# nolan-h-hamilton/ROCCO

Measured on AMD Instinct MI355X. Metric: loci/sec to converged solve, hg38 50bp K=100; BED3 intervals bit-exact, higher is better.
Workload: dtype f64

## Files before the change

rocco_amd/csrc/budget.hip:

```cpp
#include "budget.h"

#include <algorithm>
#include <atomic>
#include <chrono>
#include <cmath>
#include <cstdio>
#include <cstdlib>
#include <cstring>
#include <thread>

#include "chain.h"
#include "model_chain.h"
#include "chain_fast.h"
#include "lean.h"
#include "lean_tasks.h"
#include "search.h"

namespace rocco {

namespace {

struct DevProblem {
    const double *scores = nullptr;
    const double *costs = nullptr;
// ... 959 lines not shown
    {
        const size_t at = align_up(ls.pool_at, 256);
        if (at + bytes > ls.pool_end) {
            return nullptr;
        }
        ls.pool_at = at + bytes;
        return (char *)solver_->dev_lean_pool.ptr + at;
    }

    LeanWcapSlot wcap_slot(size_t problem) const { return lean_wcap_slot(solver_->dev_lean_wcap.ptr, probs.size(), problem); }

    void add_wcap_task(DevProblem &p, const LeanWcapSlot &slot, std::vector<LeanWcapTask> &tasks, int &blocks)
    {
        if (p.wcap_version == p.map_version) {
            return;
        }
        tasks.push_back(lean_wcap_task(p.emap, p.scores, (long long)p.n, p.qexp, p.cmax, p.sabs, slot, blocks));
        blocks += lean_tiles(p.n);
        p.wcap_version = p.map_version;
    }

    int reserve_round_scratch(long long records, bool force_fill)
    {
        DeviceBuffer &look = solver_->dev_lean_look;
        const void *old_ptr = look.ptr;
        const size_t old_bytes = look.bytes;
        int rc;
        if ((rc = look.reserve(align_up(256 + (size_t)records * 4 * sizeof(unsigned long long), 256))) != ROCCO_HIP_OK) return rc;
        if (force_fill || solver_->lean_look_dirty != 0 || look.ptr != old_ptr || look.bytes != old_bytes) {
            ROCCO_HIP_TRY(hipMemsetAsync(look.ptr, 0xFF, look.bytes, stream_));
            ROCCO_HIP_TRY(hipMemsetAsync((char *)look.ptr + 128, 0, 4, stream_));
            solver_->lean_look_dirty = 0;
        }
        return solver_->dev_lean_round.reserve(align_up((size_t)records * sizeof(LeanTileRec), 256) + 256);
    }

    LeanLaunch round_launch(const LeanTask *tasks, const double *points, LeanResult *results) const
    {
        char *look = (char *)solver_->dev_lean_look.ptr;
        LeanLaunch L;
        L.tasks = tasks;
        L.n_tasks = 0;
        L.n_units = 0;
        L.points = points;
        L.ticket = (unsigned *)look;
        L.look = (unsigned long long *)(look + 256);
        L.recs = (LeanTileRec *)solver_->dev_lean_round.ptr;
        L.bits = (unsigned *)solver_->dev_lean_pool.ptr;
        L.tile_off = (unsigned *)solver_->dev_lean_pool.ptr;
        L.results = results;
        L.error = (unsigned *)(look + 128);
        L.error_out = nullptr;
        L.self_reset = 1;
        L.pad = 0;
        L.ctl = nullptr;
        return L;
    }

    static double separator_score(double base, double gamma) { return std::floor(base - 2.0 * gamma - 2.0); }

    std::vector<std::vector<std::pair<double, long long>>> facts_;
    std::vector<std::pair<size_t, double>> open_facts_;
    bool model_chain_inflight_ = false;
    bool model_chain_running_ = false;
    int model_chain_ingested_ = 0;
    std::vector<size_t> model_chain_problems_;
    const ModelChainReport *model_chain_report_ = nullptr;
    const int *model_chain_np_ = nullptr;
    const ModelChainFact *model_chain_facts_ = nullptr;
    const ModelChainFinal *model_chain_finals_ = nullptr;
    struct Written {
        bool valid = false;
        double penalty = 0.0;
        long long count = 0;
    };
    std::vector<Written> written_;
    long long model_chain_written = 0, model_chain_windows_answered = 0;
    long long model_chains = 0, model_chain_facts = 0, model_chain_hits = 0, model_chain_misses = 0, model_chain_stopped = 0;
    long long model_tiles_answered_ = 0;
    double t_mchain_submit_ = 0.0, t_mchain_wait_ = 0.0;

    std::vector<std::pair<const char *, double>> marks_;
    bool marks_on_ = false;
    void mark(const char *label)
    {
        if (marks_on_) {
            marks_.emplace_back(label, now_us());
        }
    }

    hipEvent_t staged_event_ = nullptr;
    bool staged_pending_ = false;
    ~HipEvaluator() override
    {
        if (model_chain_running_ || !objective_pending_.empty() || objective_staged_pending_ || staged_pending_) {
            (void)hipStreamSynchronize(stream_);
        }
        if (staged_event_ != nullptr) {
            (void)hipEventDestroy(staged_event_);
        }
        if (objective_staged_event_ != nullptr) {
            (void)hipEventDestroy(objective_staged_event_);
        }
    }
    int stage_wait()
    {
        if (staged_pending_) {
// ... 2129 lines not shown
```

rocco_amd/csrc/lean.h:

```cpp
#pragma once

#include "common.h"

namespace rocco {

constexpr int kLeanChunk = 32;
constexpr int kLeanThreads = 256;
constexpr int kLeanTile = kLeanChunk * kLeanThreads;
constexpr int kLeanBatch = 8;
constexpr int kLeanMaxPoints = 64;

struct LeanTileRec {
    unsigned base;
    unsigned tail;
    unsigned cells;
    unsigned flags;
};

struct LeanTask {
    const double *s;
    long long m;
    double c_raw;
    double magic;
    double big;
    int n_tiles;
    int n_points;
    int n_groups;
    int unit_begin;
    int point_begin;
    int rec_begin;
    long long bits_begin;
    long long off_begin;
    int result_begin;
    int tile_stride;
    int independent;
    int store;
    const uint8_t *emap;
    const double *wcap;
    const unsigned *clean_chunks;
    double cmax, sabs;
    int qexp;
    int batch;
};

struct LeanResult {
    long long count;
    long long child_len;
    long long flags;
};

struct LeanRoundCtl {
    int n_tasks;
    int n_units;
    int n_pairs;
    int n_pre_tasks;
    int n_pre_blocks;
    unsigned error;
    int round;
    int all_done;
};

struct LeanLaunch {
    const LeanTask *tasks;
    int n_tasks;
    int n_units;
    const double *points;
    unsigned *ticket;
    unsigned long long *look;
    LeanTileRec *recs;
    unsigned *bits;
    unsigned *tile_off;
    LeanResult *results;
    unsigned *error;
    unsigned *error_out;
    int self_reset;
    int pad;
    LeanRoundCtl *ctl;
};

struct LeanCompactTask {
    const double *s;
    const int *orig;
    long long m;
    int n_tiles;
    int block_begin;
    const unsigned *bits;
    const unsigned *tile_off;
    double sep;
    double *out_s;
    int *out_orig;
    long long capacity;
};

struct LeanWriteTask {
    const unsigned *word1;
    const unsigned *word0;
    const unsigned *entering;
    uint8_t *solution;
    long long m;
    int n_tiles;
    int block_begin;
};
int launch_lean_write_solutions(const LeanWriteTask *tasks_dev, const int *n_tasks_dev, int grid, hipStream_t stream);

struct LeanMapOut {
    double *gain_chunk;
    double *gain_block;
};
struct LeanMapCodeTask {
    const double *gain_chunk;
    const double *gain_block;
    uint8_t *emap;
    long long m;
    double margin;
    int n_tiles;
    int block_begin;
};
int launch_lean_map(const LeanLaunch &L, const LeanMapOut &out, hipStream_t stream);
int launch_lean_mapcode(const LeanMapCodeTask *tasks_dev, int n_tasks, int n_blocks, hipStream_t stream);

int launch_lean_eval(const LeanLaunch &L, hipStream_t stream);
int launch_lean_eval_chain(const LeanLaunch &L, int grid, hipStream_t stream);
int launch_lean_finish_chain(const LeanLaunch &L, int grid, hipStream_t stream);
int launch_lean_compact_chain(const LeanCompactTask *tasks_dev, LeanRoundCtl *ctl, int grid, hipStream_t stream);
constexpr int kLeanModelBatch = 4;
int launch_lean_model(const LeanLaunch &L, hipStream_t stream);
struct LeanWcapTask {
    const uint8_t *emap;
    const double *s;
// ... 27 lines not shown
```

rocco_amd/csrc/lean.hip:

```cpp
#include "lean.h"
#include "model_chain.h"

#include <cmath>

namespace rocco {

namespace {

constexpr int kStride = kLeanChunk + 2;
constexpr int kTileLds = kLeanThreads * kStride;
constexpr unsigned long long kSentinel = ~0ull;
constexpr unsigned kSpinLimit = 1u << 22;

struct Fn {
    double a, lo, hi;
};

__device__ __forceinline__ double clampd(double x, double lo, double hi) { return fmin(fmax(x, lo), hi); }

__device__ __forceinline__ Fn compose(const Fn &f, const Fn &g)
{
    Fn r;
    r.a = f.a + g.a;
    r.lo = clampd(f.lo + g.a, g.lo, g.hi);
    r.hi = clampd(f.hi + g.a, g.lo, g.hi);
    return r;
}

__device__ __forceinline__ Fn shfl_up_fn(const Fn &f, int off)
{
    Fn r;
    r.a = __shfl_up(f.a, off);
    r.lo = __shfl_up(f.lo, off);
    r.hi = __shfl_up(f.hi, off);
    return r;
}

__device__ __forceinline__ unsigned long long granule_load(const unsigned long long *p)
{
    return __hip_atomic_load(p, __ATOMIC_RELAXED, __HIP_MEMORY_SCOPE_AGENT);
}

__device__ __forceinline__ void granule_store(unsigned long long *p, double v)
{
    __hip_atomic_store(p, (unsigned long long)__double_as_longlong(v), __ATOMIC_RELAXED, __HIP_MEMORY_SCOPE_AGENT);
}

__device__ __forceinline__ double granule_wait(const unsigned long long *p, unsigned *error)
{
    unsigned long long v = granule_load(p);
    unsigned spins = 0;
    while (v == kSentinel) {
        __builtin_amdgcn_s_sleep(2);
        v = granule_load(p);
        if (++spins > kSpinLimit) {
            atomicOr(error, 1u);
            return 0.0;
        }
    }
    return __longlong_as_double((long long)v);
}

template <typename First>
__device__ __forceinline__ int find_task(int n_tasks, int key, First first_of)
{
    const int lane = threadIdx.x & 63;
    int ti = 0;
    for (int base = 0; base < n_tasks; base += 64) {
        const int i = base + lane;
        const int v = (i < n_tasks) ? first_of(i) : 0x7FFFFFFF;
        const unsigned long long le = __ballot(v <= key);
        if (le == 0ull) {
            break;
        }
        ti = base + 63 - __builtin_clzll(le);
        if (le != ~0ull) {
            break;
        }
    }
    return ti;
}

template <bool RAW>
__device__ __forceinline__ void stage_tile(const double *__restrict__ s, long long m, long long base, double magic,
                                           double *lds)
{
    const int t = threadIdx.x;
    const bool aligned16 = ((reinterpret_cast<uintptr_t>(s) & 15U) == 0);
    if (aligned16 && base + kLeanTile <= m) {
        const double2 *__restrict__ src = reinterpret_cast<const double2 *>(s + base) + t;
        double2 v[16];
#pragma unroll
        for (int r = 0; r < 16; ++r) {
            v[r] = src[r * kLeanThreads];
        }
#pragma unroll
        for (int r = 0; r < 16; ++r) {
            const int e = 2 * (r * kLeanThreads + t);
// ... 178 lines not shown
        const bool coded = code_hz || (e - 52 < task.qexp);
        const bool hz = coded || (fabs(-x[p] - lm.nlam[p]) == lm.half_u) || gamma_tie;
        lm.hz[p] = hz;
        lm.tie[p] = hz && !coded;
        lm.c[p] = hz ? cq : cu;
        lm.w[p] = hz ? (4.0 * hb + q) : 0.0;
        lm.base[p] = hz ? (9.0 * hb + 2.0 * q) : 0.0;
    }
}

template <int PB>
__device__ __forceinline__ void chunk_function_model(const double *__restrict__ row, const double (&x)[PB],
                                                     const LaneModel<PB> &lm, bool first_unclamped, double big, Fn (&f)[PB])
{
    double lo[PB], hi[PB], fa[PB];
#pragma unroll
    for (int p = 0; p < PB; ++p) {
        fa[p] = 0.0;
        lo[p] = -big;
        hi[p] = big;
    }
#pragma unroll 1
    for (int i0 = 0; i0 < kLeanChunk; i0 += 8) {
        double rs[8];
#pragma unroll
        for (int ii = 0; ii < 8; ii += 2) {
            const double2 v = *reinterpret_cast<const double2 *>(row + i0 + ii);
            rs[ii] = v.x;
            rs[ii + 1] = v.y;
        }
#pragma unroll
        for (int ii = 0; ii < 8; ++ii) {
            const double su = (rs[ii] + lm.magic_u) - lm.magic_u;
#pragma unroll
            for (int p = 0; p < PB; ++p) {
                const double ah = ((rs[ii] - x[p]) + lm.magic_q) - lm.magic_q;
                const double a = lm.hz[p] ? ah : (su + lm.nlam[p]);
                const double cc = (first_unclamped && i0 + ii == 0) ? big : lm.c[p];
                fa[p] += a;
                lo[p] = fmin(fmax(lo[p], -cc), cc) + a;
                hi[p] = fmin(fmax(hi[p], -cc), cc) + a;
            }
        }
    }
#pragma unroll
    for (int p = 0; p < PB; ++p) {
        f[p].a = fa[p];
        f[p].lo = lo[p];
        f[p].hi = hi[p];
    }
}

template <int PB>
struct LaneTolerance {
    bool clear[PB];
    double tail[PB];
    double slack_all[PB];
    double slack_pos[PB];
    double tau_pre[PB];
    unsigned bad[PB];
};

template <int PB, bool EDGE>
__device__ __forceinline__ void chunk_classes_model(const double *__restrict__ row, const double (&x)[PB],
                                                    const LaneModel<PB> &lm, bool first_unclamped, double big,
                                                    const double (&din)[PB], int valid, int last, unsigned (&one)[PB],
                                                    unsigned (&nz)[PB], LaneTolerance<PB> &tol)
{
    double d[PB], wacc[PB];
    bool pre[PB];
    const double inf = __longlong_as_double(0x7FF0000000000000LL);
#pragma unroll
    for (int p = 0; p < PB; ++p) {
        one[p] = 0u;
        nz[p] = 0u;
        d[p] = din[p];
        wacc[p] = 0.0;
        pre[p] = true;
        tol.slack_all[p] = inf;
        tol.slack_pos[p] = inf;
        tol.tau_pre[p] = 0.0;
        tol.bad[p] = 0u;
    }
#pragma unroll 1
    for (int i0 = 0; i0 < kLeanChunk; i0 += 8) {
        double rs[8];
#pragma unroll
        for (int ii = 0; ii < 8; ii += 2) {
            const double2 v = *reinterpret_cast<const double2 *>(row + i0 + ii);
            rs[ii] = v.x;
            rs[ii + 1] = v.y;
        }
#pragma unroll
        for (int ii = 0; ii < 8; ++ii) {
            const int i = i0 + ii;
            const double su = (rs[ii] + lm.magic_u) - lm.magic_u;
            const bool exists = !EDGE || i < valid;
            const bool su_tie = exists && (fabs(rs[ii] - su) == lm.half_u);
            const bool terminal = EDGE && (i == last);
#pragma unroll
            for (int p = 0; p < PB; ++p) {
                const double ah = ((rs[ii] - x[p]) + lm.magic_q) - lm.magic_q;
                const double a = lm.hz[p] ? ah : (su + lm.nlam[p]);
                const double c = lm.c[p];
                const double cc = (first_unclamped && i == 0) ? big : c;
                d[p] = fmin(fmax(d[p], -cc), cc) + a;
                double t1 = c - d[p];
                double t2 = -c - d[p];
                if (EDGE) {
                    if (terminal) {
                        t1 = 0.0 - d[p];
                        t2 = t1;
                    }
                    if (i >= valid) {
                        t1 = 0.0;
                        t2 = 0.0;
                    }
                }
                one[p] = __builtin_amdgcn_alignbit(one[p], (unsigned)__double2hiint(t1), 31);
                nz[p] = __builtin_amdgcn_alignbit(nz[p], (unsigned)__double2hiint(t2), 31);
                const double over = fabs(d[p]) - c;
                const double margin = terminal ? fabs(d[p]) : fabs(over);
                if (exists) {
                    wacc[p] += lm.hz[p] ? lm.w[p] : (su_tie ? 2.0 * lm.half_u : 0.0);
                    const double tau = wacc[p] + lm.base[p];
                    if (pre[p]) {
                        const double slack = margin - tau;
                        tol.slack_all[p] = fmin(tol.slack_all[p], slack);
                        tol.slack_pos[p] = (tau > 0.0) ? fmin(tol.slack_pos[p], slack) : tol.slack_pos[p];
                        tol.tau_pre[p] = fmax(tol.tau_pre[p], tau);
                    } else {
                        tol.bad[p] |= (tau > kModelGuard) ? 64u : 0u;
                        tol.bad[p] |= (tau > 0.0 && !(margin > tau)) ? 1u : 0u;
                    }
                    if (!terminal && over > kModelGuard) {
                        wacc[p] = 0.0;
                        pre[p] = false;
                    }
                }
            }
        }
    }
#pragma unroll
    for (int p = 0; p < PB; ++p) {
        tol.clear[p] = !pre[p];
        tol.tail[p] = wacc[p];
        (void)valid;
    }
}

constexpr int kZeroBytes = 16384;

__global__ __launch_bounds__(256) void lean_zero_batch_kernel(const LeanScatterTask *__restrict__ tasks, int n_tasks)
{
    const int ti = find_task(n_tasks, (int)blockIdx.x, [&](int i) { return tasks[i].zero_begin; });
    const LeanScatterTask task = tasks[ti];
    const long long at = (long long)((int)blockIdx.x - task.zero_begin) * kZeroBytes;
    uint8_t *p = task.full + at;
    const long long len = min((long long)kZeroBytes, task.n - at);
    if (len == kZeroBytes && ((reinterpret_cast<uintptr_t>(p) & 15U) == 0)) {
        uint4 *q = reinterpret_cast<uint4 *>(p);
        const uint4 z = make_uint4(0u, 0u, 0u, 0u);
#pragma unroll
        for (int r = 0; r < kZeroBytes / 16 / 256; ++r) {
            q[r * 256 + threadIdx.x] = z;
        }
    } else {
        for (long long i = threadIdx.x; i < len; i += 256) {
            p[i] = 0;
        }
    }
}

__global__ __launch_bounds__(256) void lean_scatter_batch_kernel(const LeanScatterTask *__restrict__ tasks, int n_tasks)
{
    const int ti = find_task(n_tasks, (int)blockIdx.x, [&](int i) { return tasks[i].scatter_begin; });
    const LeanScatterTask task = tasks[ti];
    const long long i = (long long)((int)blockIdx.x - task.scatter_begin) * 256 + threadIdx.x;
    if (i < task.m) {
        const int o = task.orig[i];
        if (o >= 0) {
            task.full[o] = task.level_solution[i];
        }
    }
}

template <int PB, bool MODEL>
__device__ __forceinline__ void eval_body(const LeanLaunch &L, const LeanTask &task, int tile, int p0, int np, double *lds,
                                          Scratch *sc)
{
    const int t = threadIdx.x;
    const int lane = t & 63, wave = t >> 6;
    const long long base = (long long)tile * task.tile_stride * kLeanTile;
    const bool indep = task.independent != 0;

    const double c = (task.c_raw + task.magic) - task.magic;
    const double big = task.big;
    double x[PB];
#pragma unroll
    for (int p = 0; p < PB; ++p) {
        x[p] = L.points[task.point_begin + p0 + min(p, np - 1)];
    }
    const long long j0 = base + (long long)t * kLeanChunk;
    const bool first_unclamped = (j0 == 0 || (indep && t == 0));
    const double c_first = first_unclamped ? big : c;
    const double *row = lds + t * kStride;
    LaneModel<PB> lm;
    if (MODEL) {
        const long long chunk = j0 / kLeanChunk;
        const long long last_chunk = (task.m - 1) / kLeanChunk;
        lane_model<PB>(task, (int)task.emap[min(chunk, last_chunk)], x, lm);
    }

    Fn f[PB];
    if (MODEL) {
        chunk_function_model<PB>(row, x, lm, first_unclamped, big, f);
    } else {
        chunk_function<PB>(row, x, c, c_first, big, f);
    }
    Fn inc[PB];
#pragma unroll
    for (int p = 0; p < PB; ++p) {
        inc[p] = f[p];
    }
#pragma unroll
    for (int off = 1; off < 64; off <<= 1) {
#pragma unroll
        for (int p = 0; p < PB; ++p) {
            const Fn prev = shfl_up_fn(inc[p], off);
            if (lane >= off) {
                inc[p] = compose(prev, inc[p]);
            }
        }
    }
    if (lane == 63) {
#pragma unroll
        for (int p = 0; p < PB; ++p) {
            sc->wave_fn[wave][p][0] = inc[p].a;
            sc->wave_fn[wave][p][1] = inc[p].lo;
            sc->wave_fn[wave][p][2] = inc[p].hi;
        }
    }
    __syncthreads();

    if (t < np) {
        const int p = t;
        Fn agg;
        agg.a = sc->wave_fn[0][p][0];
        agg.lo = sc->wave_fn[0][p][1];
        agg.hi = sc->wave_fn[0][p][2];
#pragma unroll
        for (int w = 1; w < 4; ++w) {
            Fn g;
            g.a = sc->wave_fn[w][p][0];
            g.lo = sc->wave_fn[w][p][1];
            g.hi = sc->wave_fn[w][p][2];
            agg = compose(agg, g);
        }
        const long long rec = (long long)task.rec_begin + (long long)(p0 + p) * task.n_tiles + tile;
        unsigned long long *mine = L.look + rec * 4;
        const bool more = (tile + 1 < task.n_tiles) && !indep;
        if (more) {
            granule_store(mine + 0, agg.lo);
            granule_store(mine + 1, agg.hi);
            if (agg.lo == agg.hi) {
                granule_store(mine + 3, agg.lo);
            }
        }
        double din = 0.0;
        if (tile > 0 && !indep) {
            const unsigned long long *prev = L.look + (rec - 1) * 4;
            const double plo = granule_wait(prev + 0, L.error);
            const double phi = granule_wait(prev + 1, L.error);
            din = (plo == phi) ? plo : granule_wait(prev + 3, L.error);
        }
        sc->tile_in[p] = din;
        if (more && agg.lo != agg.hi) {
            granule_store(mine + 3, clampd(din + agg.a, agg.lo, agg.hi));
        }
    }
    __syncthreads();

    double din[PB];
#pragma unroll
    for (int p = 0; p < PB; ++p) {
        Fn e = shfl_up_fn(inc[p], 1);
        if (lane == 0) {
            e.a = 0.0;
            e.lo = -big;
            e.hi = big;
        }
        double v = sc->tile_in[min(p, np - 1)];
        for (int w = 0; w < wave; ++w) {
            v = clampd(v + sc->wave_fn[w][p][0], sc->wave_fn[w][p][1], sc->wave_fn[w][p][2]);
        }
        din[p] = clampd(v + e.a, e.lo, e.hi);
    }
    const bool edge_tile = (base + kLeanTile >= task.m);
    const int valid = (int)max(0LL, min((long long)kLeanChunk, task.m - j0));
    const int last = (task.m - 1 >= j0 && task.m - 1 < j0 + kLeanChunk) ? (int)(task.m - 1 - j0) : -1;
    unsigned one[PB], nz[PB];
    if (MODEL) {
        LaneTolerance<PB> tol;
        if (edge_tile) {
            chunk_classes_model<PB, true>(row, x, lm, first_unclamped, big, din, valid, last, one, nz, tol);
        } else {
            chunk_classes_model<PB, false>(row, x, lm, first_unclamped, big, din, valid, last, one, nz, tol);
        }
        const double wcap = *task.wcap;
        const double q_step = ldexp(1.0, task.qexp);
        const int e_gamma = tie_exponent(task.c_raw);
#pragma unroll
        for (int p = 0; p < PB; ++p) {
            double extra = 0.0;
            const int e_lam = tie_exponent(x[p]);
            if (e_lam + kModelMapBias >= 0 && e_lam + kModelMapBias < 128) {
                const unsigned chunks = task.clean_chunks[e_lam + kModelMapBias];
                const double hb = ldexp(1.0, e_lam + 2 - 53);
                extra += (chunks != 0u) ? (double)chunks * (double)kLeanChunk * (4.0 * hb + q_step) + 9.0 * hb + 2.0 * q_step : 0.0;
            }
            if (e_gamma != e_lam && e_gamma + kModelMapBias >= 0 && e_gamma + kModelMapBias < 128) {
                const unsigned chunks = task.clean_chunks[e_gamma + kModelMapBias];
                const double hb = ldexp(1.0, e_gamma + 2 - 53);
                extra += (chunks != 0u) ? (double)chunks * (double)kLeanChunk * (4.0 * hb + q_step) + 9.0 * hb + 2.0 * q_step : 0.0;
            }
            const double wave_in = (base == 0 && wave == 0) ? 0.0 : wcap + extra;
            bool cl = tol.clear[p];
            double tl = tol.tail[p];
#pragma unroll
            for (int off = 1; off < 64; off <<= 1) {
                const int pc = __shfl_up((int)cl, off);
                const double pt = __shfl_up(tl, off);
                if (lane >= off) {
                    tl = cl ? tl : pt + tl;
                    cl = cl || (pc != 0);
                }
            }
            int ec = __shfl_up((int)cl, 1);
            double et = __shfl_up(tl, 1);
            if (lane == 0) {
                ec = 0;
                et = 0.0;
            }
            const double w_in = ec ? et : wave_in + et;
            unsigned why = tol.bad[p];
            why |= (w_in + tol.tau_pre[p] > kModelGuard) ? 2u : 0u;
            why |= (w_in > 0.0 && !(tol.slack_all[p] > w_in)) ? 4u : 0u;
            why |= !(tol.slack_pos[p] > w_in) ? 8u : 0u;
            if (p >= np) {
                why = 0u;
            }
#pragma unroll
            for (int off = 32; off > 0; off >>= 1) {
                why |= __shfl_xor(why, off);
            }
            if (why != 0u && lane == 0) {
                atomicOr(&sc->uncertain[p], why);
            }
        }
    } else if (edge_tile) {
        chunk_classes<PB, true>(row, x, c, c_first, din, valid, last, one, nz);
    } else {
        chunk_classes<PB, false>(row, x, c, c_first, din, valid, last, one, nz);
    }

    unsigned zw[PB];
    bool dep[PB];
    unsigned cnt0[PB], tail[PB];
#pragma unroll
    for (int p = 0; p < PB; ++p) {
        const unsigned det = one[p] | ~nz[p];
        const bool pass = (det == 0u);
        tail[p] = pass ? 32u : (unsigned)__builtin_ctz(det);
        const unsigned long long sum0 = (unsigned long long)nz[p] + (unsigned long long)one[p];
        const unsigned z0 = (unsigned)((sum0 ^ nz[p] ^ one[p]) >> 1);
        cnt0[p] = (unsigned)__builtin_popcount(z0);
        const bool v = (z0 >> 31) != 0u;
        const unsigned long long pass_b = __ballot(pass), v_b = __ballot(v);
        const unsigned long long right = (lane == 63) ? 0ull : (~pass_b & (~0ull << (lane + 1)));
        const bool in_wave = (right != 0ull);
        const unsigned zin_wave = in_wave ? (unsigned)((v_b >> __builtin_ctzll(right)) & 1ull) : 0u;
        if (lane == 0) {
            sc->wave_pass[wave][p] = (unsigned char)(pass_b == ~0ull);
            sc->wave_v[wave][p] = (pass_b == ~0ull) ? 0 : (unsigned char)((v_b >> __builtin_ctzll(~pass_b)) & 1ull);
        }
        zw[p] = zin_wave;
        dep[p] = !in_wave;
    }
    __syncthreads();
    unsigned cells_lane[PB];
#pragma unroll
    for (int p = 0; p < PB; ++p) {
        unsigned zin = zw[p];
        bool d = dep[p];
        if (d) {
            for (int w = wave + 1; w < 4; ++w) {
                if (!sc->wave_pass[w][p]) {
                    zin = sc->wave_v[w][p];
                    d = false;
                    break;
                }
            }
        }
        dep[p] = d;
        const unsigned zeff = d ? 1u : zin;
        const unsigned long long sum = (unsigned long long)nz[p] + (unsigned long long)one[p] + zeff;
        zw[p] = (unsigned)((sum ^ nz[p] ^ one[p]) >> 1);
        if (MODEL && task.store == 2 && p < np) {
            const unsigned long long sum0 = (unsigned long long)nz[p] + (unsigned long long)one[p] + (d ? 0u : zin);
            const unsigned z_if0 = (unsigned)((sum0 ^ nz[p] ^ one[p]) >> 1);
            const long long plane = (long long)task.n_points * task.n_tiles * kLeanThreads;
            const long long at = task.bits_begin + ((long long)(p0 + p) * task.n_tiles + tile) * kLeanThreads + t;
            L.bits[at] = zw[p];
            L.bits[at + plane] = z_if0;
        }
        if (!d) {
            cnt0[p] += tail[p] * zin;
            tail[p] = 0u;
        }
        if (lane == 0) {
            sc->first_word[wave][p] = zw[p];
        }
        if (t == kLeanThreads - 1) {
            sc->last_word[p] = zw[p];
        }
    }
    __syncthreads();
#pragma unroll
    for (int p = 0; p < PB; ++p) {
        unsigned nxt = __shfl_down(zw[p], 1);
        if (lane == 63) {
            nxt = (wave < 3) ? sc->first_word[wave + 1][p] : 0x80000000u;
        }
        unsigned ends = zw[p] & ~((zw[p] << 1) | (nxt >> 31));
        if (last >= 0) {
            ends &= ~(0x80000000u >> last);
        }
        cells_lane[p] = (unsigned)__builtin_popcount(zw[p]) + (unsigned)__builtin_popcount(ends);
    }

#pragma unroll
    for (int p = 0; p < PB; ++p) {
        unsigned b = cnt0[p], tl = tail[p], ce = cells_lane[p];
#pragma unroll
        for (int off = 32; off > 0; off >>= 1) {
            b += __shfl_down(b, off);
            tl += __shfl_down(tl, off);
            ce += __shfl_down(ce, off);
        }
        if (lane == 0 && p < np) {
            atomicAdd(&sc->red[p][0], b);
            atomicAdd(&sc->red[p][1], tl);
            atomicAdd(&sc->red[p][2], ce);
        }
        if (p < np && task.store == 1) {
            L.bits[task.bits_begin + ((long long)(p0 + p) * task.n_tiles + tile) * kLeanThreads + t] = zw[p];
        }
    }
    __syncthreads();
    if (t < np) {
        const int p = t;
        bool all_pass = true;
        unsigned v = 0u;
        for (int w = 0; w < 4; ++w) {
            if (!sc->wave_pass[w][p]) {
                all_pass = false;
                v = sc->wave_v[w][p];
                break;
            }
        }
        LeanTileRec r;
        r.base = sc->red[p][0];
        r.tail = sc->red[p][1];
        r.cells = sc->red[p][2];
        const unsigned firstw = sc->first_word[0][p];
        r.flags = (all_pass ? 1u : 0u) | (v << 1) | ((firstw >> 31) << 2) | ((sc->last_word[p] & 1u) << 3) |
                  (MODEL ? (sc->uncertain[p] << 4) : 0u);
        L.recs[(long long)task.rec_begin + (long long)(p0 + p) * task.n_tiles + tile] = r;
    }
}

__device__ __forceinline__ void finish_pair(const LeanLaunch &L, int n_tasks, int pair)
{
    const int lane = threadIdx.x;
    int ti = 0, acc = 0;
    for (int base = 0; base < n_tasks; base += 64) {
        const int i = base + lane;
        const int np_i = (i < n_tasks) ? L.tasks[i].n_points : 0;
        int incl = np_i;
#pragma unroll
        for (int off = 1; off < 64; off <<= 1) {
            const int v = __shfl_up(incl, off);
            incl += (lane >= off) ? v : 0;
        }
        const unsigned long long beyond = __ballot(i < n_tasks && acc + incl > pair);
        if (beyond != 0ull) {
            const int at = __builtin_ctzll(beyond);
            ti = base + at;
            acc += __shfl(incl - np_i, at);
            break;
        }
        acc += __shfl(incl, 63);
        ti = min(n_tasks - 1, base + 63);
    }
    const LeanTask task = L.tasks[ti];
    const int p = pair - acc;
// ... 291 lines not shown
        r.cells = 0u;
        r.flags = 1u;
        L.recs[rec] = r;
    }
    __syncthreads();
    Fn e = shfl_up_fn(inc, 1);
    if (lane == 0) {
        e.a = 0.0;
        e.lo = -big;
        e.hi = big;
    }
    double v = sc->tile_in[0];
    for (int w = 0; w < wave; ++w) {
        v = clampd(v + sc->wave_fn[w][0][0], sc->wave_fn[w][0][1], sc->wave_fn[w][0][2]);
    }
    double d = clampd(v + e.a, e.lo, e.hi);
    double g = 0.0;
    for (int i = 0; i < valid; ++i) {
        const double a = ((row[i] - lam) + magic) - magic;
        if (j0 + i > 0) {
            g += fmax(0.0, d - c);
            d = fmin(fmax(d, -c), c) + a;
        } else {
            d = a;
        }
    }
    const long long rec = (long long)task.rec_begin + tile;
    out.gain_chunk[rec * kLeanThreads + t] = g;
    double gs = g;
#pragma unroll
    for (int off = 32; off > 0; off >>= 1) {
        gs += __shfl_down(gs, off);
    }
    __syncthreads();
    if (lane == 0) {
        sc->wave_fn[wave][1][0] = gs;
    }
    __syncthreads();
    if (t == 0) {
        out.gain_block[rec] = ((sc->wave_fn[0][1][0] + sc->wave_fn[1][1][0]) + sc->wave_fn[2][1][0]) + sc->wave_fn[3][1][0];
    }
}

__global__ __launch_bounds__(kLeanThreads, 2) void lean_map_kernel(LeanLaunch L, LeanMapOut out)
{
    extern __shared__ __attribute__((aligned(16))) double smem[];
    double *lds = smem;
    Scratch *sc = reinterpret_cast<Scratch *>(smem + kTileLds);
    const int t = threadIdx.x;
    if (t == 0) {
        sc->ticket = (int)(atomicAdd(L.ticket, 1u) + 1u);
    }
    __syncthreads();
    const int ticket = sc->ticket;
    if (ticket >= L.n_units) {
        return;
    }
    const int ti = find_task(L.n_tasks, ticket, [&](int i) { return L.tasks[i].unit_begin; });
    const LeanTask task = L.tasks[ti];
    const int tile = ticket - task.unit_begin;
    stage_tile<true>(task.s, task.m, (long long)tile * kLeanTile, task.magic, lds);
    map_body(L, task, tile, lds, sc, out);
}

__device__ __forceinline__ uint8_t lean_binade_code(double p0_lo, double p0_hi, double margin)
{
    const double top = fmax(p0_hi, 1.0);
    int e = ilogb(top);
    if (e > 60) {
        e = 60;
    }
    bool clean = false;
    if (p0_lo > 0.0) {
        const double lo_edge = ldexp(1.0, e), hi_edge = ldexp(1.0, e + 1);
        clean = (p0_lo - lo_edge > margin) && (hi_edge - p0_hi > margin);
    }
    return (uint8_t)((clean ? 0 : 0x80) | (e + kModelMapBias));
}

__global__ __launch_bounds__(kLeanThreads) void lean_mapcode_kernel(const LeanMapCodeTask *__restrict__ tasks, int n_tasks)
{
    __shared__ double wsum[4];
    __shared__ double pre_s;
    const int ti = find_task(n_tasks, (int)blockIdx.x, [&](int i) { return tasks[i].block_begin; });
    const LeanMapCodeTask task = tasks[ti];
    const int tile = (int)blockIdx.x - task.block_begin;
    const int lane = threadIdx.x & 63, wave = threadIdx.x >> 6;
    if (wave == 0) {
        double carry = 0.0;
        for (int base = 0; base <= tile; base += 64) {
            const int b = base + lane;
            const double g = (b < task.n_tiles) ? task.gain_block[b] : 0.0;
            double inc = g;
#pragma unroll
            for (int off = 1; off < 64; off <<= 1) {
                const double p = __shfl_up(inc, off);
                if (lane >= off) {
                    inc += p;
                }
            }
            if (b == tile) {
                pre_s = carry + (inc - g);
            }
            carry += __shfl(inc, 63);
        }
    }
    const long long chunk = (long long)tile * kLeanThreads + threadIdx.x;
// ... 45 lines not shown
            for (int q = 0; q < 4; ++q) {
                unsigned v = 0u;
#pragma unroll
                for (int b = 0; b < 4; ++b) {
                    v |= ((z >> (31 - (4 * q + b))) & 1u) << (8 * b);
                }
                w[q] = v;
            }
            w = reinterpret_cast<unsigned *>(&hi);
#pragma unroll
            for (int q = 0; q < 4; ++q) {
                unsigned v = 0u;
#pragma unroll
                for (int b = 0; b < 4; ++b) {
                    v |= ((z >> (31 - (16 + 4 * q + b))) & 1u) << (8 * b);
                }
                w[q] = v;
            }
            *reinterpret_cast<uint4 *>(task.solution + j0) = lo;
            *reinterpret_cast<uint4 *>(task.solution + j0 + 16) = hi;
        } else {
            for (int b = 0; b < kLeanChunk && j0 + b < task.m; ++b) {
                task.solution[j0 + b] = (uint8_t)((z >> (31 - b)) & 1u);
            }
        }
    }
}

__global__ __launch_bounds__(256) void lean_scatter_kernel(const uint8_t *__restrict__ level, const int *__restrict__ orig,
                                                           long long m, uint8_t *__restrict__ full)
{
    const long long i = (long long)blockIdx.x * 256 + threadIdx.x;
    if (i < m) {
        const int o = orig[i];
        if (o >= 0) {
            full[o] = level[i];
        }
    }
}

__global__ __launch_bounds__(kLeanThreads, 2) void lean_eval_kernel(LeanLaunch L)
{
    extern __shared__ __attribute__((aligned(16))) double smem[];
    double *lds = smem;
    Scratch *sc = reinterpret_cast<Scratch *>(smem + kTileLds);
    const int t = threadIdx.x;
    if (t == 0) {
        sc->ticket = (int)(atomicAdd(L.ticket, 1u) + 1u);
    }
    if (t < kLeanBatch * 4) {
        (&sc->red[0][0])[t] = 0u;
    }
    __syncthreads();
    const int ticket = sc->ticket;
    if (ticket >= L.n_units) {
        return;
    }
    const int ti = find_task(L.n_tasks, ticket, [&](int i) { return L.tasks[i].unit_begin; });
    const LeanTask task = L.tasks[ti];
    const int unit = ticket - task.unit_begin;
    const int tile = unit / task.n_groups, group = unit % task.n_groups;
    const int p0 = group * task.batch;
    const int np = min(task.batch, task.n_points - p0);
    stage_tile<false>(task.s, task.m, (long long)tile * task.tile_stride * kLeanTile, task.magic, lds);
    if (np > 4) {
        eval_body<8, false>(L, task, tile, p0, np, lds, sc);
    } else if (np > 2) {
        eval_body<4, false>(L, task, tile, p0, np, lds, sc);
    } else if (np > 1) {
        eval_body<2, false>(L, task, tile, p0, np, lds, sc);
    } else {
        eval_body<1, false>(L, task, tile, p0, np, lds, sc);
    }
}

__global__ __launch_bounds__(kLeanThreads, 2) void lean_eval_chain_kernel(LeanLaunch L)
{
    extern __shared__ __attribute__((aligned(16))) double smem[];
    double *lds = smem;
    Scratch *sc = reinterpret_cast<Scratch *>(smem + kTileLds);
    const int t = threadIdx.x;
    const int n_units = L.ctl->n_units, n_tasks = L.ctl->n_tasks;
    if (n_units <= 0) {
        return;
    }
    for (;;) {
        if (t == 0) {
            sc->ticket = (int)(atomicAdd(L.ticket, 1u) + 1u);
        }
        if (t < kLeanBatch * 4) {
            (&sc->red[0][0])[t] = 0u;
        }
        __syncthreads();
        const int ticket = sc->ticket;
        if (ticket >= n_units) {
            return;
        }
        const int ti = find_task(n_tasks, ticket, [&](int i) { return L.tasks[i].unit_begin; });
        const LeanTask task = L.tasks[ti];
        const int unit = ticket - task.unit_begin;
        const int tile = unit / task.n_groups, group = unit % task.n_groups;
        const int p0 = group * task.batch;
        const int np = min(task.batch, task.n_points - p0);
        stage_tile<false>(task.s, task.m, (long long)tile * task.tile_stride * kLeanTile, task.magic, lds);
        if (np > 4) {
            eval_body<8, false>(L, task, tile, p0, np, lds, sc);
        } else if (np > 2) {
            eval_body<4, false>(L, task, tile, p0, np, lds, sc);
        } else if (np > 1) {
            eval_body<2, false>(L, task, tile, p0, np, lds, sc);
        } else {
            eval_body<1, false>(L, task, tile, p0, np, lds, sc);
        }
        __syncthreads();
    }
}

__global__ __launch_bounds__(kLeanThreads, 2) void lean_model_kernel(LeanLaunch L)
{
    extern __shared__ __attribute__((aligned(16))) double smem[];
    double *lds = smem;
    Scratch *sc = reinterpret_cast<Scratch *>(smem + kTileLds);
    const int t = threadIdx.x;
    if (t == 0) {
        sc->ticket = (int)(atomicAdd(L.ticket, 1u) + 1u);
    }
    if (t < kLeanBatch * 4) {
        (&sc->red[0][0])[t] = 0u;
    }
    if (t < kLeanBatch) {
        sc->uncertain[t] = 0u;
    }
    __syncthreads();
    const int ticket = sc->ticket;
    if (ticket >= L.n_units) {
        return;
    }
    const int ti = find_task(L.n_tasks, ticket, [&](int i) { return L.tasks[i].unit_begin; });
    const LeanTask task = L.tasks[ti];
    const int unit = ticket - task.unit_begin;
    const int tile = unit / task.n_groups, group = unit % task.n_groups;
    const int p0 = group * task.batch;
    const int np = min(task.batch, task.n_points - p0);
    stage_tile<true>(task.s, task.m, (long long)tile * kLeanTile, task.magic, lds);
    if (np > 2) {
        eval_body<4, true>(L, task, tile, p0, np, lds, sc);
    } else if (np > 1) {
        eval_body<2, true>(L, task, tile, p0, np, lds, sc);
    } else {
        eval_body<1, true>(L, task, tile, p0, np, lds, sc);
    }
}

__global__ __launch_bounds__(kLeanThreads, 2) void lean_model_chain_kernel(LeanLaunch L)
{
    extern __shared__ __attribute__((aligned(16))) double smem[];
    double *lds = smem;
    Scratch *sc = reinterpret_cast<Scratch *>(smem + kTileLds);
    const int t = threadIdx.x;
    const int n_units = L.ctl->n_units, n_tasks = L.ctl->n_tasks;
    if (n_units <= 0) {
        return;
    }
    for (;;) {
        if (t == 0) {
            sc->ticket = (int)(atomicAdd(L.ticket, 1u) + 1u);
        }
        if (t < kLeanBatch * 4) {
            (&sc->red[0][0])[t] = 0u;
        }
        if (t < kLeanBatch) {
            sc->uncertain[t] = 0u;
        }
        __syncthreads();
        const int ticket = sc->ticket;
        if (ticket >= n_units) {
            return;
        }
        const int ti = find_task(n_tasks, ticket, [&](int i) { return L.tasks[i].unit_begin; });
        const LeanTask task = L.tasks[ti];
        const int unit = ticket - task.unit_begin;
        const int tile = unit / task.n_groups, group = unit % task.n_groups;
        const int p0 = group * task.batch;
        const int np = min(task.batch, task.n_points - p0);
        stage_tile<true>(task.s, task.m, (long long)tile * kLeanTile, task.magic, lds);
        if (np > 2) {
            eval_body<4, true>(L, task, tile, p0, np, lds, sc);
        } else if (np > 1) {
            eval_body<2, true>(L, task, tile, p0, np, lds, sc);
        } else {
            eval_body<1, true>(L, task, tile, p0, np, lds, sc);
        }
        __syncthreads();
    }
}

__global__ __launch_bounds__(kLeanThreads) void lean_wcap_count_kernel(const LeanWcapTask *__restrict__ tasks, int n_tasks)
{
    __shared__ unsigned steps[128], ties[128], clean[128];
    __shared__ double magic_u[kLeanThreads], half_u[kLeanThreads];
    const int ti = find_task(n_tasks, (int)blockIdx.x, [&](int i) { return tasks[i].block_begin; });
    const LeanWcapTask task = tasks[ti];
    const int t = threadIdx.x;
    if (t < 128) {
        steps[t] = 0u;
        ties[t] = 0u;
        clean[t] = 0u;
    }
    __syncthreads();
    const long long base = (long long)((int)blockIdx.x - task.block_begin) * kLeanTile;
    const long long n_chunks = (task.m + kLeanChunk - 1) / kLeanChunk;
    const long long chunk = base / kLeanChunk + t;
    int my_bin = 0;
    magic_u[t] = 0.0;
    half_u[t] = 0.0;
    if (chunk < n_chunks) {
        const int code = task.emap[chunk];
        int e = (code & 0x7F) - kModelMapBias;
        const bool code_hz = (code & 0x80) != 0;
        if (code_hz) {
            e = max(e, task.e_floor);
        }
        my_bin = min(max(e + kModelMapBias, 0), 127);
        if (code_hz || e - 52 < task.qexp) {
            atomicAdd(&steps[my_bin], (unsigned)kLeanChunk);
        } else {
            magic_u[t] = ldexp(1.5, e);
            half_u[t] = ldexp(1.0, e - 53);
// ... 243 lines not shown
```

Measured before the change: 5.676 billion.

## Add clean-wave fast paths and DPP lane ops to lean model eval

Adds specialized model-chunk function and class routines for waves with no hz lanes, no edge tiles and (optionally) no rounding ties, which skip the per-element general tolerance bookkeeping. Replaces the off-by-one shuffles with DPP row-shift ops and replaces the shuffle reductions with a DPP wave sum that packs two 16-bit counts per word. Also makes the ticket wave-uniform with readfirstlane and shrinks the unroll of the general class loop from 8 to 4. The risks are 16-bit overflow in the packed sums, DPP row shifts not crossing 16-lane rows, and correctness of the simplified uncertainty checks. A new env flag can force the general path.

```diff
diff --git a/rocco_amd/csrc/budget.hip b/rocco_amd/csrc/budget.hip
--- a/rocco_amd/csrc/budget.hip
+++ b/rocco_amd/csrc/budget.hip
@@ -1035,7 +1035,7 @@
         L.error = (unsigned *)(look + 128);
         L.error_out = nullptr;
         L.self_reset = 1;
-        L.pad = 0;
+        L.model_general = env_flag("ROCCO_HIP_LEAN_MODEL_GENERAL", false) ? 1 : 0;
         L.ctl = nullptr;
         return L;
     }
diff --git a/rocco_amd/csrc/lean.h b/rocco_amd/csrc/lean.h
--- a/rocco_amd/csrc/lean.h
+++ b/rocco_amd/csrc/lean.h
@@ -74,7 +74,7 @@
     unsigned *error;
     unsigned *error_out;
     int self_reset;
-    int pad;
+    int model_general;
     LeanRoundCtl *ctl;
 };
 
diff --git a/rocco_amd/csrc/lean.hip b/rocco_amd/csrc/lean.hip
--- a/rocco_amd/csrc/lean.hip
+++ b/rocco_amd/csrc/lean.hip
@@ -36,6 +36,24 @@
     return r;
 }
 
+__device__ __forceinline__ int lane_below(int v) { return __builtin_amdgcn_update_dpp(v, v, 0x138, 0xF, 0xF, false); }
+
+__device__ __forceinline__ double lane_below(double v)
+{
+    return __hiloint2double(lane_below(__double2hiint(v)), lane_below(__double2loint(v)));
+}
+
+__device__ __forceinline__ int lane_above(int v) { return __builtin_amdgcn_update_dpp(v, v, 0x130, 0xF, 0xF, false); }
+
+__device__ __forceinline__ Fn lane_below_fn(const Fn &f)
+{
+    Fn r;
+    r.a = lane_below(f.a);
+    r.lo = lane_below(f.lo);
+    r.hi = lane_below(f.hi);
+    return r;
+}
+
 __device__ __forceinline__ unsigned long long granule_load(const unsigned long long *p)
 {
     return __hip_atomic_load(p, __ATOMIC_RELAXED, __HIP_MEMORY_SCOPE_AGENT);
@@ -44,6 +62,16 @@
 __device__ __forceinline__ void granule_store(unsigned long long *p, double v)
 {
     __hip_atomic_store(p, (unsigned long long)__double_as_longlong(v), __ATOMIC_RELAXED, __HIP_MEMORY_SCOPE_AGENT);
+}
+
+__device__ __forceinline__ unsigned wave_sum(unsigned v)
+{
+    v += (unsigned)__builtin_amdgcn_update_dpp(0, (int)v, 0x111, 0xF, 0xF, true);
+    v += (unsigned)__builtin_amdgcn_update_dpp(0, (int)v, 0x112, 0xF, 0xF, true);
+    v += (unsigned)__builtin_amdgcn_update_dpp(0, (int)v, 0x114, 0xF, 0xF, true);
+    v += (unsigned)__builtin_amdgcn_update_dpp(0, (int)v, 0x118, 0xF, 0xF, true);
+    return (unsigned)__builtin_amdgcn_readlane((int)v, 15) + (unsigned)__builtin_amdgcn_readlane((int)v, 31) +
+           (unsigned)__builtin_amdgcn_readlane((int)v, 47) + (unsigned)__builtin_amdgcn_readlane((int)v, 63);
 }
 
 __device__ __forceinline__ double granule_wait(const unsigned long long *p, unsigned *error)
@@ -328,6 +356,52 @@
 }
 
 template <int PB>
+__device__ __forceinline__ bool chunk_function_model_clean(const double *__restrict__ row, const LaneModel<PB> &lm,
+                                                           double c_raw, bool first_unclamped, double big, Fn (&f)[PB])
+{
+    double lo[PB], hi[PB], fa[PB];
+#pragma unroll
+    for (int p = 0; p < PB; ++p) {
+        fa[p] = 0.0;
+        lo[p] = -big;
+        hi[p] = big;
+    }
+    const double c = (c_raw + lm.magic_u) - lm.magic_u;
+    const double c0 = first_unclamped ? big : c;
+    bool tie = false;
+#pragma unroll 1
+    for (int i0 = 0; i0 < kLeanChunk; i0 += 8) {
+        double rs[8];
+#pragma unroll
+        for (int ii = 0; ii < 8; ii += 2) {
+            const double2 v = *reinterpret_cast<const double2 *>(row + i0 + ii);
+            rs[ii] = v.x;
+            rs[ii + 1] = v.y;
+        }
+#pragma unroll
+        for (int ii = 0; ii < 8; ++ii) {
+            const double su = (rs[ii] + lm.magic_u) - lm.magic_u;
+            tie = tie || (fabs(rs[ii] - su) == lm.half_u);
+            const double cc = (ii == 0 && i0 == 0) ? c0 : c;
+#pragma unroll
+            for (int p = 0; p < PB; ++p) {
+                const double a = su + lm.nlam[p];
+                fa[p] += a;
+                lo[p] = fmin(fmax(lo[p], -cc), cc) + a;
+                hi[p] = fmin(fmax(hi[p], -cc), cc) + a;
+            }
+        }
+    }
+#pragma unroll
+    for (int p = 0; p < PB; ++p) {
+        f[p].a = fa[p];
+        f[p].lo = lo[p];
+        f[p].hi = hi[p];
+    }
+    return tie;
+}
+
+template <int PB>
 struct LaneTolerance {
     bool clear[PB];
     double tail[PB];
@@ -359,16 +433,16 @@
         tol.bad[p] = 0u;
     }
 #pragma unroll 1
-    for (int i0 = 0; i0 < kLeanChunk; i0 += 8) {
-        double rs[8];
-#pragma unroll
-        for (int ii = 0; ii < 8; ii += 2) {
+    for (int i0 = 0; i0 < kLeanChunk; i0 += 4) {
+        double rs[4];
+#pragma unroll
+        for (int ii = 0; ii < 4; ii += 2) {
             const double2 v = *reinterpret_cast<const double2 *>(row + i0 + ii);
             rs[ii] = v.x;
             rs[ii + 1] = v.y;
         }
 #pragma unroll
-        for (int ii = 0; ii < 8; ++ii) {
+        for (int ii = 0; ii < 4; ++ii) {
             const int i = i0 + ii;
             const double su = (rs[ii] + lm.magic_u) - lm.magic_u;
             const bool exists = !EDGE || i < valid;
@@ -425,6 +499,129 @@
     }
 }
 
+template <int PB>
+__device__ __forceinline__ void chunk_classes_model_clean(const double *__restrict__ row, const LaneModel<PB> &lm,
+                                                          double c_raw, bool first_unclamped, double big,
+                                                          const double (&din)[PB],
+                                                          unsigned (&one)[PB], unsigned (&nz)[PB], bool (&clear)[PB],
+                                                          double (&slack_all)[PB])
+{
+    double d[PB];
+    bool pre[PB];
+    const double inf = __longlong_as_double(0x7FF0000000000000LL);
+    const double c = (c_raw + lm.magic_u) - lm.magic_u, nc = -c;
+    const double c0 = first_unclamped ? big : c;
+#pragma unroll
+    for (int p = 0; p < PB; ++p) {
+        one[p] = 0u;
+        nz[p] = 0u;
+        d[p] = din[p];
+        pre[p] = true;
+        slack_all[p] = inf;
+    }
+#pragma unroll 1
+    for (int i0 = 0; i0 < kLeanChunk; i0 += 8) {
+        double rs[8];
+#pragma unroll
+        for (int ii = 0; ii < 8; ii += 2) {
+            const double2 v = *reinterpret_cast<const double2 *>(row + i0 + ii);
+            rs[ii] = v.x;
+            rs[ii + 1] = v.y;
+        }
+#pragma unroll
+        for (int ii = 0; ii < 8; ++ii) {
+            const double su = (rs[ii] + lm.magic_u) - lm.magic_u;
+            const double cc = (ii == 0 && i0 == 0) ? c0 : c;
+#pragma unroll
+            for (int p = 0; p < PB; ++p) {
+                const double a = su + lm.nlam[p];
+                d[p] = fmin(fmax(d[p], -cc), cc) + a;
+                const double t1 = c - d[p];
+                const double t2 = nc - d[p];
+                one[p] = __builtin_amdgcn_alignbit(one[p], (unsigned)__double2hiint(t1), 31);
+                nz[p] = __builtin_amdgcn_alignbit(nz[p], (unsigned)__double2hiint(t2), 31);
+                const double over = fabs(d[p]) - c;
+                slack_all[p] = fmin(slack_all[p], pre[p] ? fabs(over) : inf);
+                pre[p] = pre[p] && !(over > kModelGuard);
+            }
+        }
+    }
+#pragma unroll
+    for (int p = 0; p < PB; ++p) {
+        clear[p] = !pre[p];
+    }
+}
+
+template <int PB>
+__device__ __forceinline__ void chunk_classes_model_ties(const double *__restrict__ row, const LaneModel<PB> &lm,
+                                                         double c_raw, bool first_unclamped, double big,
+                                                         const double (&din)[PB], unsigned (&one)[PB], unsigned (&nz)[PB],
+                                                         LaneTolerance<PB> &tol)
+{
+    double d[PB], wacc[PB], gate[PB], slack_post[PB], tau_post[PB];
+    const double inf = __longlong_as_double(0x7FF0000000000000LL);
+    const double c = (c_raw + lm.magic_u) - lm.magic_u, nc = -c;
+    const double c0 = first_unclamped ? big : c;
+    const double u = 2.0 * lm.half_u;
+#pragma unroll
+    for (int p = 0; p < PB; ++p) {
+        one[p] = 0u;
+        nz[p] = 0u;
+        d[p] = din[p];
+        wacc[p] = 0.0;
+        gate[p] = -inf;
+        slack_post[p] = inf;
+        tau_post[p] = 0.0;
+        tol.slack_all[p] = inf;
+        tol.slack_pos[p] = inf;
+        tol.tau_pre[p] = 0.0;
+    }
+#pragma unroll 1
+    for (int i0 = 0; i0 < kLeanChunk; i0 += 8) {
+        double rs[8];
+#pragma unroll
+        for (int ii = 0; ii < 8; ii += 2) {
+            const double2 v = *reinterpret_cast<const double2 *>(row + i0 + ii);
+            rs[ii] = v.x;
+            rs[ii + 1] = v.y;
+        }
+#pragma unroll
+        for (int ii = 0; ii < 8; ++ii) {
+            const double su = (rs[ii] + lm.magic_u) - lm.magic_u;
+            const double step = (fabs(rs[ii] - su) == lm.half_u) ? u : 0.0;
+            const double cc = (ii == 0 && i0 == 0) ? c0 : c;
+#pragma unroll
+            for (int p = 0; p < PB; ++p) {
+                const double a = su + lm.nlam[p];
+                d[p] = fmin(fmax(d[p], -cc), cc) + a;
+                const double t1 = c - d[p];
+                const double t2 = nc - d[p];
+                one[p] = __builtin_amdgcn_alignbit(one[p], (unsigned)__double2hiint(t1), 31);
+                nz[p] = __builtin_amdgcn_alignbit(nz[p], (unsigned)__double2hiint(t2), 31);
+                const double over = fabs(d[p]) - c;
+                wacc[p] += step;
+                const double tau = wacc[p];
+                const double slack = fabs(over) - tau;
+                const double slack_w = (tau > 0.0) ? slack : inf;
+                tol.slack_all[p] = fmin(tol.slack_all[p], fmax(slack, gate[p]));
+                tol.slack_pos[p] = fmin(tol.slack_pos[p], fmax(slack_w, gate[p]));
+                tol.tau_pre[p] = fmax(tol.tau_pre[p], fmin(tau, -gate[p]));
+                slack_post[p] = fmin(slack_post[p], fmax(slack_w, -gate[p]));
+                tau_post[p] = fmax(tau_post[p], fmin(tau, gate[p]));
+                const bool clamps = over > kModelGuard;
+                wacc[p] = clamps ? 0.0 : wacc[p];
+                gate[p] = clamps ? inf : gate[p];
+            }
+        }
+    }
+#pragma unroll
+    for (int p = 0; p < PB; ++p) {
+        tol.clear[p] = gate[p] > 0.0;
+        tol.tail[p] = wacc[p];
+        tol.bad[p] = ((tau_post[p] > kModelGuard) ? 64u : 0u) | (!(slack_post[p] > 0.0) ? 1u : 0u);
+    }
+}
+
 constexpr int kZeroBytes = 16384;
 
 __global__ __launch_bounds__(256) void lean_zero_batch_kernel(const LeanScatterTask *__restrict__ tasks, int n_tasks)
@@ -482,15 +679,26 @@
     const double c_first = first_unclamped ? big : c;
     const double *row = lds + t * kStride;
     LaneModel<PB> lm;
+    bool clean_wave = false, su_tie = false;
     if (MODEL) {
         const long long chunk = j0 / kLeanChunk;
         const long long last_chunk = (task.m - 1) / kLeanChunk;
         lane_model<PB>(task, (int)task.emap[min(chunk, last_chunk)], x, lm);
+        bool hz_any = false;
+#pragma unroll
+        for (int p = 0; p < PB; ++p) {
+            hz_any = hz_any || lm.hz[p];
+        }
+        clean_wave = (L.model_general == 0) && (__ballot(hz_any) == 0ull);
     }
 
     Fn f[PB];
     if (MODEL) {
-        chunk_function_model<PB>(row, x, lm, first_unclamped, big, f);
+        if (clean_wave) {
+            su_tie = chunk_function_model_clean<PB>(row, lm, task.c_raw, first_unclamped, big, f);
+        } else {
+            chunk_function_model<PB>(row, x, lm, first_unclamped, big, f);
+        }
     } else {
         chunk_function<PB>(row, x, c, c_first, big, f);
     }
@@ -503,7 +711,7 @@
     for (int off = 1; off < 64; off <<= 1) {
 #pragma unroll
         for (int p = 0; p < PB; ++p) {
-            const Fn prev = shfl_up_fn(inc[p], off);
+            const Fn prev = (off == 1) ? lane_below_fn(inc[p]) : shfl_up_fn(inc[p], off);
             if (lane >= off) {
                 inc[p] = compose(prev, inc[p]);
             }
@@ -560,7 +768,7 @@
     double din[PB];
 #pragma unroll
     for (int p = 0; p < PB; ++p) {
-        Fn e = shfl_up_fn(inc[p], 1);
+        Fn e = lane_below_fn(inc[p]);
         if (lane == 0) {
             e.a = 0.0;
             e.lo = -big;
@@ -577,8 +785,16 @@
     const int last = (task.m - 1 >= j0 && task.m - 1 < j0 + kLeanChunk) ? (int)(task.m - 1 - j0) : -1;
     unsigned one[PB], nz[PB];
     if (MODEL) {
+        const bool clean_tile = clean_wave && (__ballot(edge_tile) == 0ull);
+        const bool clean_classes = clean_tile && (__ballot(su_tie) == 0ull);
         LaneTolerance<PB> tol;
-        if (edge_tile) {
+        bool clean_clear[PB];
+        double clean_slack[PB];
+        if (clean_classes) {
+            chunk_classes_model_clean<PB>(row, lm, task.c_raw, first_unclamped, big, din, one, nz, clean_clear, clean_slack);
+        } else if (clean_tile) {
+            chunk_classes_model_ties<PB>(row, lm, task.c_raw, first_unclamped, big, din, one, nz, tol);
+        } else if (edge_tile) {
             chunk_classes_model<PB, true>(row, x, lm, first_unclamped, big, din, valid, last, one, nz, tol);
         } else {
             chunk_classes_model<PB, false>(row, x, lm, first_unclamped, big, din, valid, last, one, nz, tol);
@@ -586,6 +802,7 @@
         const double wcap = *task.wcap;
         const double q_step = ldexp(1.0, task.qexp);
         const int e_gamma = tie_exponent(task.c_raw);
+        double wave_in[PB];
 #pragma unroll
         for (int p = 0; p < PB; ++p) {
             double extra = 0.0;
@@ -600,7 +817,24 @@
                 const double hb = ldexp(1.0, e_gamma + 2 - 53);
                 extra += (chunks != 0u) ? (double)chunks * (double)kLeanChunk * (4.0 * hb + q_step) + 9.0 * hb + 2.0 * q_step : 0.0;
             }
-            const double wave_in = (base == 0 && wave == 0) ? 0.0 : wcap + extra;
+            wave_in[p] = (base == 0 && wave == 0) ? 0.0 : wcap + extra;
+        }
+        if (clean_classes) {
+#pragma unroll
+            for (int p = 0; p < PB; ++p) {
+                const unsigned long long clear_b = __ballot(clean_clear[p]);
+                const bool ec = (clear_b & ((1ull << lane) - 1ull)) != 0ull;
+                const double w_in = ec ? 0.0 : wave_in[p];
+                const bool why2 = (w_in > kModelGuard) && (p < np);
+                const bool why4 = (w_in > 0.0 && !(clean_slack[p] > w_in)) && (p < np);
+                const unsigned why = (__ballot(why2) != 0ull ? 2u : 0u) | (__ballot(why4) != 0ull ? 4u : 0u);
+                if (why != 0u && lane == 0) {
+                    atomicOr(&sc->uncertain[p], why);
+                }
+            }
+        } else {
+#pragma unroll
+        for (int p = 0; p < PB; ++p) {
             bool cl = tol.clear[p];
             double tl = tol.tail[p];
 #pragma unroll
@@ -618,7 +852,7 @@
                 ec = 0;
                 et = 0.0;
             }
-            const double w_in = ec ? et : wave_in + et;
+            const double w_in = ec ? et : wave_in[p] + et;
             unsigned why = tol.bad[p];
             why |= (w_in + tol.tau_pre[p] > kModelGuard) ? 2u : 0u;
             why |= (w_in > 0.0 && !(tol.slack_all[p] > w_in)) ? 4u : 0u;
@@ -633,6 +867,7 @@
             if (why != 0u && lane == 0) {
                 atomicOr(&sc->uncertain[p], why);
             }
+        }
         }
     } else if (edge_tile) {
         chunk_classes<PB, true>(row, x, c, c_first, din, valid, last, one, nz);
@@ -704,7 +939,7 @@
     __syncthreads();
 #pragma unroll
     for (int p = 0; p < PB; ++p) {
-        unsigned nxt = __shfl_down(zw[p], 1);
+        unsigned nxt = (unsigned)lane_above((int)zw[p]);
         if (lane == 63) {
             nxt = (wave < 3) ? sc->first_word[wave + 1][p] : 0x80000000u;
         }
@@ -715,19 +950,22 @@
         cells_lane[p] = (unsigned)__builtin_popcount(zw[p]) + (unsigned)__builtin_popcount(ends);
     }
 
-#pragma unroll
-    for (int p = 0; p < PB; ++p) {
-        unsigned b = cnt0[p], tl = tail[p], ce = cells_lane[p];
-#pragma unroll
-        for (int off = 32; off > 0; off >>= 1) {
-            b += __shfl_down(b, off);
-            tl += __shfl_down(tl, off);
-            ce += __shfl_down(ce, off);
-        }
+    unsigned cells_sum[PB];
+#pragma unroll
+    for (int p = 0; p < PB; p += 2) {
+        const unsigned packed = wave_sum(cells_lane[p] | ((p + 1 < PB) ? (cells_lane[p + 1] << 16) : 0u));
+        cells_sum[p] = packed & 0xFFFFu;
+        if (p + 1 < PB) {
+            cells_sum[p + 1] = packed >> 16;
+        }
+    }
+#pragma unroll
+    for (int p = 0; p < PB; ++p) {
+        const unsigned packed = wave_sum(cnt0[p] | (tail[p] << 16));
         if (lane == 0 && p < np) {
-            atomicAdd(&sc->red[p][0], b);
-            atomicAdd(&sc->red[p][1], tl);
-            atomicAdd(&sc->red[p][2], ce);
+            atomicAdd(&sc->red[p][0], packed & 0xFFFFu);
+            atomicAdd(&sc->red[p][1], packed >> 16);
+            atomicAdd(&sc->red[p][2], cells_sum[p]);
         }
         if (p < np && task.store == 1) {
             L.bits[task.bits_begin + ((long long)(p0 + p) * task.n_tiles + tile) * kLeanThreads + t] = zw[p];
@@ -1125,7 +1363,7 @@
         sc->ticket = (int)(atomicAdd(L.ticket, 1u) + 1u);
     }
     __syncthreads();
-    const int ticket = sc->ticket;
+    const int ticket = __builtin_amdgcn_readfirstlane(sc->ticket);
     if (ticket >= L.n_units) {
         return;
     }
@@ -1277,7 +1515,7 @@
         (&sc->red[0][0])[t] = 0u;
     }
     __syncthreads();
-    const int ticket = sc->ticket;
+    const int ticket = __builtin_amdgcn_readfirstlane(sc->ticket);
     if (ticket >= L.n_units) {
         return;
     }
@@ -1317,7 +1555,7 @@
             (&sc->red[0][0])[t] = 0u;
         }
         __syncthreads();
-        const int ticket = sc->ticket;
+        const int ticket = __builtin_amdgcn_readfirstlane(sc->ticket);
         if (ticket >= n_units) {
             return;
         }
@@ -1357,7 +1595,7 @@
         sc->uncertain[t] = 0u;
     }
     __syncthreads();
-    const int ticket = sc->ticket;
+    const int ticket = __builtin_amdgcn_readfirstlane(sc->ticket);
     if (ticket >= L.n_units) {
         return;
     }
@@ -1398,7 +1636,7 @@
             sc->uncertain[t] = 0u;
         }
         __syncthreads();
-        const int ticket = sc->ticket;
+        const int ticket = __builtin_amdgcn_readfirstlane(sc->ticket);
         if (ticket >= n_units) {
             return;
         }
```

After: 5.564 billion. 0.98x the previous value.
